# 0411tony/Yue

Hardware: AMD Instinct MI355X
Metric: BPR triplet-updates/sec at k=128 (S-round semantics, user rows sequential; the reference's exact sequential semantics: secondary.exact) (higher is better)
Workload: dtype f32

## Files before the change

### yue_amd/csrc/bpr_host.hip

```cpp
#include "host_common.hpp"

#include "train_kernels.hpp"
#include "round_kernels.hpp"

using yue_host::fail;
using yue_host::kr_of;
using yue_host::with_kr;
static_assert(yue::kNllSlots == yue_host::kNllSlotsHost && yue::kHeaderSlack == yue_host::kHeaderSlackHost &&
              yue::kMetaStageMax == (uint32_t)yue_host::kMetaStageMaxHost, "host_common.hpp mirrors these");

namespace {

yue::TrainArgs make_args(yue_ctx *c, double lr, double regU, double regI) {
    yue::TrainArgs a{};
    a.P = c->P.p; a.Q = c->Q.p; a.dP = c->dP.p; a.dQ = c->dQ.p;
    a.stage = c->Q.p ? c->Q.p + (size_t)c->n * c->k : nullptr;
    a.ev_u = c->ev_u.p; a.ev_i = c->ev_i.p; a.ev_j = c->ev_j.p;
    a.indptr = c->indptr.p; a.indices = c->indices.p;
    a.nll_slots = c->scal.p;
    a.m = c->m; a.n = c->n; a.k = c->k;
    a.lr = lr;
    a.ru = (float)(lr * regU);
    a.ri = (float)(lr * regI);
    a.neg_lo = 0; a.neg_range = (int32_t)c->n;
    return a;
}

void launch_level(yue_ctx *c, const yue::TrainArgs &a, int64_t e0, int64_t e1) {
    const int tpw = (int)std::min<int64_t>(64, std::max<int64_t>(1, (e1 - e0) / 4096));
    const int64_t waves = (e1 - e0 + tpw - 1) / tpw;
    const dim3 grid((unsigned)((waves + 3) / 4)), block(256);
    with_kr(c->k, [&](auto kr) { hipLaunchKernelGGL(yue::k_bpr_level<kr()>, grid, block, 0, c->stream, a, e0, e1, tpw); });
}

constexpr int kRoundInstances[][2] = {{1, 8}, {1, 16}, {2, 8}, {4, 4}, {1, 4}, {2, 4}, {1, 2}, {2, 2}};

constexpr int default_round_tpw(int kr, bool meta) { return kr == 4 ? 4 : kr == 2 ? 8 : meta ? 8 : 16; }

template <class F, size_t... I>
bool with_round_instance(int kr, int tpw, F &&f, std::index_sequence<I...>) {
    return ((kr == kRoundInstances[I][0] && tpw == kRoundInstances[I][1] &&
             (f(std::integral_constant<int, kRoundInstances[I][0]>{}, std::integral_constant<int, kRoundInstances[I][1]>{}), true)) || ...);
}
template <class F>
bool with_round_instance(int kr, int tpw, F &&f) {
    return with_round_instance(kr, tpw, f, std::make_index_sequence<sizeof kRoundInstances / sizeof kRoundInstances[0]>{});
}

int tpw_of(const yue_ctx *c, bool meta) { return c->opt_round_tpw ? c->opt_round_tpw : default_round_tpw(kr_of(c->k), meta); }

constexpr int64_t kMetaRangeMax = 37 * 1024;
constexpr int64_t kMetaRangesMax = 12;
constexpr int64_t kRoundGenerationsMax = 6;
constexpr double kRoundEventsPerItemRow = 4.0;

bool meta_bucketed(const yue_ctx *c) { return c->n > kMetaRangeMax * kMetaRangesMax || c->opt_round_bucket; }
bool meta_path_fits(const yue_ctx *c) { return c->opt_round_meta && c->n <= ((int64_t)yue::kBucketRangesMax << yue::kBucketShift); }

int default_round_events(yue_ctx *c, double n_rows, int64_t *out) {
    const bool fold = yue_host::fold_path(c);
    const int tpw = tpw_of(c, fold);
    int per_cu = 0, cus = 0;
    hipError_t e = hipSuccess;
    if (!with_round_instance(kr_of(c->k), tpw, [&](auto kr, auto t) {
            e = fold ? hipOccupancyMaxActiveBlocksPerMultiprocessor(&per_cu, yue::k_round_m<kr(), t()>, 256, 0)
                     : hipOccupancyMaxActiveBlocksPerMultiprocessor(&per_cu, yue::k_round<kr(), t()>, 256, 0);
        }))
        return fail(YUE_ERR_ARG, "unsupported (k, TPW) combination");
    HIPCHK(e);
    per_cu = std::min(per_cu, fold ? 7 : 6);
    HIPCHK(hipDeviceGetAttribute(&cus, hipDeviceAttributeMultiprocessorCount, c->device));
    const double slots = (double)per_cu * (double)cus;
    int64_t w = (int64_t)(slots * 4.0 * tpw);
    w -= w % 1024;
    w = std::max<int64_t>(w, 1024);
    if (fold) {
        int64_t sets = std::min<int64_t>(kRoundGenerationsMax, std::max<int64_t>(1, (int64_t)(kRoundEventsPerItemRow * n_rows / (double)w)));
        if (2.0 * (double)(w * sets) < 2.0 * n_rows) sets = std::min<int64_t>(sets, 4);
        w *= sets;
    }
    *out = w;
    return YUE_OK;
}

int launch_round(yue_ctx *c, const yue::TrainArgs &a_in, int64_t e0, int64_t e1, int64_t n0, int64_t n1,
                 int parity, int apply_p) {
    unsigned long long *cnt[2] = {c->cnt0.p, c->cnt1.p};
    uint32_t *cntp[2] = {c->cntp0.p, c->cntp1.p};
    yue::RoundArgs ra{};
    ra.e_begin = e0; ra.e_end = e1; ra.n_begin = n0; ra.n_end = n1;
    ra.cnt_cur = cnt[parity]; ra.cnt_next = cnt[parity ^ 1]; ra.cntp_cur = cntp[parity]; ra.cntp_next = cntp[parity ^ 1];
    uint32_t *tab[2] = {c->tab0.p, c->tab1.p};
    ra.tab_cur = tab[parity]; ra.tab_next = tab[parity ^ 1]; ra.staged = c->staged ? 1 : 0;
    ra.apply_p = apply_p;
    const int tpw = tpw_of(c, false);
    const int64_t waves = (std::max(e1 - e0, n1 - n0) + tpw - 1) / tpw;
    const int64_t blocks = (waves + 3) / 4;
    if (blocks == 0) return YUE_OK;
    const dim3 grid((unsigned)blocks), block(256);
#ifdef YUE_STAMPS
    yue::TrainArgs a = a_in;
    a.stamps = nullptr;
    if (e1 > e0 && c->update_launches++ == c->stamp_launch) {
        HIPCHK(c->stamps.resize((size_t)waves * 8));
        HIPCHK(hipMemsetAsync(c->stamps.p, 0, (size_t)waves * 64, c->stream));
        a.stamps = c->stamps.p;
        c->stamp_waves = (e1 - e0 + tpw - 1) / tpw;
    }
#else
    const yue::TrainArgs &a = a_in;
#endif
    if (!with_round_instance(kr_of(c->k), tpw, [&](auto kr, auto t) {
            hipLaunchKernelGGL((yue::k_round<kr(), t()>), grid, block, 0, c->stream, a, ra, a.ev_u, a.ev_i, a.ev_j);
        }))
        return fail(YUE_ERR_ARG, "unsupported (k, TPW) combination");
    return YUE_OK;
}

int launch_round_meta(yue_ctx *c, const yue::TrainArgs &a, const std::vector<int64_t> &bounds) {
    const int64_t R = (int64_t)bounds.size() - 1;
    const int64_t E = bounds.back();
    HIPCHK(c->meta_i.resize((size_t)E + yue::kHeaderSlack)); HIPCHK(c->meta_j.resize((size_t)E + yue::kHeaderSlack));
    HIPCHK(c->round_rows.resize((size_t)R)); HIPCHK(c->d_bounds.resize((size_t)R + 1));
    if (c->h_bounds != bounds) {
        HIPCHK(hipStreamSynchronize(c->stream));
        c->h_bounds = bounds;
        HIPCHK(hipMemcpyAsync(c->d_bounds.p, c->h_bounds.data(), (size_t)(R + 1) * sizeof(int64_t), hipMemcpyHostToDevice, c->stream));
    }
    HIPCHK(hipMemsetAsync(c->round_rows.p, 0, (size_t)R * sizeof(unsigned long long), c->stream));
    HIPCHK(c->fold.resize((size_t)(E + 4 * R + 8)));
    yue::MetaArgs ma{};
    ma.ev_i = a.ev_i; ma.ev_j = a.ev_j; ma.bounds = c->d_bounds.p; ma.R = R; ma.n = (int32_t)c->n;
    const bool bucketed = meta_bucketed(c);
    if (bucketed) {
        ma.range = 1 << yue::kBucketShift;
        ma.G = (int32_t)((c->n + ma.range - 1) >> yue::kBucketShift);
        HIPCHK(c->bk_touch.resize((size_t)(2 * E + 2))); HIPCHK(c->bk_ptr.resize((size_t)R * (ma.G + 1)));
        yue::BucketArgs ba{};
        ba.ev_i = a.ev_i; ba.ev_j = a.ev_j; ba.bounds = c->d_bounds.p; ba.R = R; ba.G = ma.G;
        ba.bk_touch = c->bk_touch.p; ba.bk_ptr = c->bk_ptr.p; ba.meta_i = c->meta_i.p; ba.meta_j = c->meta_j.p;
        int cus0 = 0;
        HIPCHK(hipDeviceGetAttribute(&cus0, hipDeviceAttributeMultiprocessorCount, c->device));
        hipLaunchKernelGGL(yue::k_round_bucket, dim3((unsigned)std::min<int64_t>(R, 2 * cus0)), dim3(1024), 0, c->stream, ba);
        ma.bk_touch = c->bk_touch.p; ma.bk_ptr = c->bk_ptr.p;
    } else {
        ma.G = (int32_t)((c->n + kMetaRangeMax - 1) / kMetaRangeMax);
        ma.range = (int32_t)((c->n + ma.G - 1) / ma.G);
    }
    ma.chunk = (ma.range + 1023) / 1024; ma.chunk |= 1;
    int64_t widest = 0;
    for (int64_t r = 0; r < R; ++r) widest = std::max(widest, bounds[(size_t)r + 1] - bounds[(size_t)r]);
    const double mean_touches = 2.0 * (double)widest / (double)std::max<int64_t>(1, c->n);
    const uint32_t stage_auto = (uint32_t)std::min<double>((double)yue::kMetaStageMax, std::max<double>((double)yue::kMetaStageDefault,
                                                         std::ceil(mean_touches * (kr_of(c->k) == 1 ? 4.0 : 2.0))));
    ma.stage_max = !c->staged ? 1u : c->opt_round_stage >= 2 ? (uint32_t)c->opt_round_stage : stage_auto;
    c->last_stage_max = (int)ma.stage_max;
    ma.meta_i = c->meta_i.p; ma.meta_j = c->meta_j.p; ma.round_rows = c->round_rows.p; ma.fold = c->fold.p;
    const size_t lds = (size_t)ma.range * sizeof(uint32_t);
    const void *kfn = bucketed ? (const void *)yue::k_round_meta<true> : (const void *)yue::k_round_meta<false>;
    HIPCHK(hipFuncSetAttribute(kfn, hipFuncAttributeMaxDynamicSharedMemorySize, (int)lds));
    int per_cu = 0, cus = 0;
    if (bucketed) { HIPCHK(hipOccupancyMaxActiveBlocksPerMultiprocessor(&per_cu, yue::k_round_meta<true>, 1024, lds)); }
    else { HIPCHK(hipOccupancyMaxActiveBlocksPerMultiprocessor(&per_cu, yue::k_round_meta<false>, 1024, lds)); }
    HIPCHK(hipDeviceGetAttribute(&cus, hipDeviceAttributeMultiprocessorCount, c->device));
    const int64_t grid = std::max<int64_t>(8, std::min<int64_t>((R * ma.G + 7) / 8 * 8, (int64_t)std::max(per_cu, 1) * cus / 8 * 8));
    if (bucketed) hipLaunchKernelGGL(yue::k_round_meta<true>, dim3((unsigned)grid), dim3(1024), lds, c->stream, ma);
    else
        hipLaunchKernelGGL(yue::k_round_meta<false>, dim3((unsigned)grid), dim3(1024), lds, c->stream, ma);
    HIPCHK(hipGetLastError());
    return YUE_OK;
}

void launch_round_fold(yue_ctx *c, const yue::TrainArgs &a, int64_t e0, int64_t e1, int64_t round_index) {
    yue::FoldArgs f{};
    f.fold = c->fold.p + yue::fold_base(e0, round_index); f.round_rows = c->round_rows.p + round_index; f.Q = a.Q; f.dQ = a.dQ; f.stage = a.stage; f.k = c->k; f.capacity = (uint32_t)((e1 - e0) & ~(int64_t)3);
    const dim3 fgrid((unsigned)std::min<int64_t>(c->opt_fold_blocks, std::max<int64_t>(1, (e1 - e0 + 15) / 16))), block(256);
    with_kr(c->k, [&](auto kr) { hipLaunchKernelGGL(yue::k_round_fold<kr()>, fgrid, block, 0, c->stream, f); });
}

int launch_round_m(yue_ctx *c, const yue::TrainArgs &a_in, int64_t e0, int64_t e1, int64_t round_index) {
    yue::RoundMArgs ra{};
    ra.e_begin = e0; ra.e_end = e1; ra.staged = c->staged ? 1 : 0;
    const int tpw = tpw_of(c, true);
    const int64_t waves = (e1 - e0 + tpw - 1) / tpw;
    const int64_t blocks = (waves + 3) / 4;
    if (blocks == 0) return YUE_OK;
    const dim3 grid((unsigned)blocks), block(256);
#ifdef YUE_STAMPS
    yue::TrainArgs a = a_in;
    a.stamps = nullptr;
    if (c->update_launches++ == c->stamp_launch) {
        HIPCHK(c->stamps.resize((size_t)waves * 8));
        HIPCHK(hipMemsetAsync(c->stamps.p, 0, (size_t)waves * 64, c->stream));
        a.stamps = c->stamps.p;
        c->stamp_waves = waves;
    }
#else
    const yue::TrainArgs &a = a_in;
#endif
    const uint32_t *mi = c->meta_i.p, *mj = c->meta_j.p;
    if (c->bigq) {
        bool is_default = false;
        with_round_instance(kr_of(c->k), tpw, [&](auto kr, auto t) {
            if constexpr (t() == default_round_tpw(kr(), true)) {
// ... 8 lines not shown
        return fail(YUE_ERR_ARG, "unsupported (k, TPW) combination");
    launch_round_fold(c, a, e0, e1, round_index);
    return YUE_OK;
}

int launch_round_u(yue_ctx *c, const yue::TrainArgs &a, int64_t u0, int64_t u1, int64_t e0, int64_t e1, int64_t round_index) {
    yue::RoundUArgs ra{};
    ra.u_begin = u0; ra.u_end = u1; ra.ev_ptr = c->d_ev_ptr.p; ra.e_begin = e0; ra.e_end = e1; ra.staged = c->staged ? 1 : 0; ra.margins = c->margins.p;
    ra.psq_slots = c->psq_in_rounds ? c->psq_slots.p : nullptr;
    const int64_t blocks = (u1 - u0 + 3) / 4;
    if (blocks == 0) return YUE_OK;
    const dim3 grid((unsigned)blocks), block(256);
    const uint32_t *mi = c->meta_i.p, *mj = c->meta_j.p;
    with_kr(c->k, [&](auto kr) {
        if (c->opt_round_fast) hipLaunchKernelGGL((yue::k_round_u<kr(), true>), grid, block, 0, c->stream, a, ra, a.ev_i, a.ev_j, mi, mj);
        else hipLaunchKernelGGL((yue::k_round_u<kr(), false>), grid, block, 0, c->stream, a, ra, a.ev_i, a.ev_j, mi, mj);
    });
    launch_round_fold(c, a, e0, e1, round_index);
    return YUE_OK;
}

template <typename F>
int run_rounds(yue_ctx *c, yue::TrainArgs a, const std::vector<int64_t> &bounds, int apply_p, F after_round, bool meta = false, const std::vector<int64_t> *user_blocks = nullptr) {
    const int64_t R = (int64_t)bounds.size() - 1;
    int64_t widest = 0;
    for (int64_t r = 0; r < R; ++r) widest = std::max(widest, bounds[(size_t)r + 1] - bounds[(size_t)r]);
    if (widest >= (1ll << 24)) meta = false;
    const bool fits31 = (c->n + 2 * widest) * (int64_t)c->k * 4 < (1ll << 31);
    c->bigq = meta && !fits31;
    if (!meta && (int64_t)c->n * c->k * 4 >= (1ll << 31))
        return fail(YUE_ERR_ARG, "item matrices of 2 GiB and more per GPU are supported by yue_bpr_epoch's default path only (not by explicit rounds / round_meta = 0 / rounds of 2^24 events and more)");
    c->staged = c->opt_round_stage && widest > 0 && (fits31 || c->bigq);
    if (c->staged) {
        const size_t need = (size_t)(c->n + 2 * widest) * (size_t)c->k;
        if (c->Q.n < need) {
            DevBuf<float> bigger;
            HIPCHK(bigger.resize(need));
            HIPCHK(hipMemcpyAsync(bigger.p, c->Q.p, (size_t)c->n * c->k * sizeof(float), hipMemcpyDeviceToDevice, c->stream));
            HIPCHK(hipStreamSynchronize(c->stream));
            c->Q.release();
            c->Q = bigger;
            a.Q = c->Q.p;
        }
        if (!meta) {
            HIPCHK(c->tab0.resize((size_t)c->n * yue::kStageMax));
            HIPCHK(c->tab1.resize((size_t)c->n * yue::kStageMax));
        }
        a.stage = c->Q.p + (size_t)c->n * c->k;
    }
    std::vector<int64_t> ne;
    for (int64_t r = 0; r < R; ++r) if (bounds[(size_t)r + 1] > bounds[(size_t)r]) ne.push_back(r);
    int rc;
    if (meta) {
        if (!ne.empty() && (rc = launch_round_meta(c, a, bounds))) return rc;
    } else if (!ne.empty()) {
        const int64_t r0 = ne[0];
        if ((rc = launch_round(c, a, 0, 0, bounds[(size_t)r0], bounds[(size_t)r0 + 1], 1, apply_p))) return rc;
    }
    const bool timed = c->timing_stride > 0 && !ne.empty();
    if (timed) {
        if (c->ev_used == c->ev_pool.size()) {
            hipEvent_t s, t;
            HIPCHK(hipEventCreate(&s));
            HIPCHK(hipEventCreate(&t));
            c->ev_pool.emplace_back(s, t);
            c->ev_triplets.push_back(0);
            c->ev_launches.push_back(0);
        }
        HIPCHK(hipEventRecord(c->ev_pool[c->ev_used].first, c->stream));
    }
    size_t pos = 0;
    for (int64_t r = 0; r < R; ++r) {
        if (pos < ne.size() && ne[pos] == r) {
            const int64_t e0 = bounds[(size_t)r], e1 = bounds[(size_t)r + 1];
            int64_t n0 = 0, n1 = 0;
            if (pos + 1 < ne.size()) { n0 = bounds[(size_t)ne[pos + 1]]; n1 = bounds[(size_t)ne[pos + 1] + 1]; }
            const bool seq_user = meta && user_blocks && !c->bigq;
            if ((rc = seq_user ? launch_round_u(c, a, (*user_blocks)[(size_t)r], (*user_blocks)[(size_t)r + 1], e0, e1, r)
                      : meta ? launch_round_m(c, a, e0, e1, r) : launch_round(c, a, e0, e1, n0, n1, (int)(pos & 1), apply_p))) return rc;
            ++pos;
        }
        if ((rc = after_round(r))) return rc;
    }
    if (timed) {
        HIPCHK(hipEventRecord(c->ev_pool[c->ev_used].second, c->stream));
        c->ev_triplets[c->ev_used] = bounds.back() - bounds.front();
        c->ev_launches[c->ev_used] = (int64_t)ne.size();
        c->ev_used++;
    }
    return YUE_OK;
}

void reset_round_state(yue_ctx *c) {
    (void)hipStreamSynchronize(c->stream);
    if (c->cnt0.p) (void)hipMemsetAsync(c->cnt0.p, 0, c->cnt0.n * sizeof(unsigned long long), c->stream);
    if (c->cnt1.p) (void)hipMemsetAsync(c->cnt1.p, 0, c->cnt1.n * sizeof(unsigned long long), c->stream);
    if (c->cntp0.p) (void)hipMemsetAsync(c->cntp0.p, 0, c->cntp0.n * sizeof(uint32_t), c->stream);
    if (c->cntp1.p) (void)hipMemsetAsync(c->cntp1.p, 0, c->cntp1.n * sizeof(uint32_t), c->stream);
    if (c->dP.p) (void)hipMemsetAsync(c->dP.p, 0, c->dP.n * sizeof(float), c->stream);
    if (c->dQ.p) (void)hipMemsetAsync(c->dQ.p, 0, c->dQ.n * sizeof(float), c->stream);
    (void)hipStreamSynchronize(c->stream);
}

}

namespace yue_host {
bool fold_path(const yue_ctx *c) { return meta_path_fits(c); }
// ... 155 lines not shown
    HIPCHK(hipStreamSynchronize(c->stream));
    return YUE_OK;
}

int yue_adam_reset(yue_ctx *c) {
    if (!c || !c->have_factors) return fail(YUE_ERR_ARG, "yue_adam_reset: no factors uploaded");
    HIPCHK(hipSetDevice(c->device));
    const size_t mk = (size_t)c->m * c->k, nk = (size_t)c->n * c->k;
    HIPCHK(c->aU_m.resize(mk)); HIPCHK(c->aU_v.resize(mk)); HIPCHK(c->aV_m.resize(nk)); HIPCHK(c->aV_v.resize(nk));
    HIPCHK(hipMemsetAsync(c->aU_m.p, 0, mk * sizeof(float), c->stream)); HIPCHK(hipMemsetAsync(c->aU_v.p, 0, mk * sizeof(float), c->stream));
    HIPCHK(hipMemsetAsync(c->aV_m.p, 0, nk * sizeof(float), c->stream)); HIPCHK(hipMemsetAsync(c->aV_v.p, 0, nk * sizeof(float), c->stream));
    HIPCHK(hipMemsetAsync(c->dP.p, 0, mk * sizeof(float), c->stream)); HIPCHK(hipMemsetAsync(c->dQ.p, 0, nk * sizeof(float), c->stream));
    c->adam_m = c->m; c->adam_n = c->n; c->adam_k = c->k;
    return YUE_OK;
}

int yue_adam_get_moments(yue_ctx *c, float *mU, float *vU, float *mV, float *vV) {
    if (!c || !c->have_factors || c->adam_m != c->m || c->adam_n != c->n || c->adam_k != c->k)
        return fail(YUE_ERR_ARG, "yue_adam_get_moments: no Adam state for the uploaded factors");
    HIPCHK(hipSetDevice(c->device));
    HIPCHK(hipStreamSynchronize(c->stream));
    const size_t mk = (size_t)c->m * c->k * sizeof(float), nk = (size_t)c->n * c->k * sizeof(float);
    if (mU) HIPCHK(hipMemcpy(mU, c->aU_m.p, mk, hipMemcpyDeviceToHost));
    if (vU) HIPCHK(hipMemcpy(vU, c->aU_v.p, mk, hipMemcpyDeviceToHost));
    if (mV) HIPCHK(hipMemcpy(mV, c->aV_m.p, nk, hipMemcpyDeviceToHost));
    if (vV) HIPCHK(hipMemcpy(vV, c->aV_v.p, nk, hipMemcpyDeviceToHost));
    return YUE_OK;
}

int yue_adam_step(yue_ctx *c, const int32_t *u, const int32_t *i, const int32_t *j, int64_t T, double lr, double reg, int64_t step, double *loss_out) {
    if (!c || !c->have_factors) return fail(YUE_ERR_ARG, "yue_adam_step: no factors uploaded");
    if (T <= 0 || !u || !i || !j || step < 1) return fail(YUE_ERR_ARG, "yue_adam_step: bad argument (T > 0, step >= 1)");
    HIPCHK(hipSetDevice(c->device));
    if (c->adam_m != c->m || c->adam_n != c->n || c->adam_k != c->k) { const int rc0 = yue_adam_reset(c); if (rc0) return rc0; }
    for (int64_t t = 0; t < T; ++t)
        if (u[t] < 0 || u[t] >= c->m || i[t] < 0 || i[t] >= c->n || j[t] < 0 || j[t] >= c->n) return fail(YUE_ERR_ARG, "yue_adam_step: triplet " + std::to_string(t) + " out of range");
    int rc = upload_triplets(c, u, i, j, T, true);
    if (rc) return rc;
    if ((rc = zero_scalars(c))) return rc;
    yue::MbArgs a{};
    a.U = c->P.p; a.V = c->Q.p; a.gU = c->dP.p; a.gV = c->dQ.p; a.k = c->k; a.u = c->xu.p; a.i = c->xi.p; a.j = c->xj.p; a.T = T;
    a.reg = (float)reg; a.loss_slots = c->scal.p;
    const dim3 grid((unsigned)(((T + 31) / 32 + 3) / 4));
    with_kr(c->k, [&](auto kr) { hipLaunchKernelGGL(yue::k_mb_grad<kr()>, grid, dim3(256), 0, c->stream, a); });
    if ((rc = yue_host::adam_apply(c, lr, step))) return rc;
    return read_scalars(c, loss_out, nullptr, nullptr);
}

int yue_sample_negatives(yue_ctx *c, uint64_t seed, uint32_t epoch, int32_t *j_out) {
    if (!c || !c->have_inter || !j_out) return fail(YUE_ERR_ARG, "yue_sample_negatives: no interactions uploaded");
    HIPCHK(hipSetDevice(c->device));
    yue::TrainArgs a = make_args(c, 0, 0, 0);
    a.seed = seed; a.epoch = epoch;
    if (c->E > 0) {
        hipLaunchKernelGGL(yue::k_sample, dim3((unsigned)((c->E + 255) / 256)), dim3(256), 0, c->stream, a, c->E);
        HIPCHK(hipGetLastError());
        HIPCHK(hipMemcpyAsync(j_out, c->ev_j.p, c->E * sizeof(int32_t), hipMemcpyDeviceToHost, c->stream));
    }
    HIPCHK(hipStreamSynchronize(c->stream));
    return YUE_OK;
}

int yue_sumsq(yue_ctx *c, double *sp, double *sq) {
    if (!c || !c->have_factors) return fail(YUE_ERR_ARG, "yue_sumsq: no factors uploaded");
    HIPCHK(hipSetDevice(c->device));
    int rc = sumsq_async(c);
    if (rc) return rc;
    double h[2];
    HIPCHK(hipMemcpyAsync(h, c->scal.p + yue::kNllSlots + 1, sizeof h, hipMemcpyDeviceToHost, c->stream));
    HIPCHK(hipStreamSynchronize(c->stream));
    if (sp) *sp = h[0];
    if (sq) *sq = h[1];
    return YUE_OK;
}

int yue_bpr_epoch(yue_ctx *c, uint64_t seed, uint32_t epoch, int64_t round_events, double lr, double regU, double regI,
                  double *nll_out, double *sumsqP_out, double *sumsqQ_out) {
    if (!c || !c->have_factors || !c->have_inter) return fail(YUE_ERR_ARG, "yue_bpr_epoch: upload factors and interactions first");
    if (round_events < 0) return fail(YUE_ERR_ARG, "yue_bpr_epoch: round_events must be positive (or 0 for the device's default)");
    HIPCHK(hipSetDevice(c->device));
    yue::TrainArgs a = make_args(c, lr, regU, regI);
    a.seed = seed + 0x632BE59BD9B4E019ull * (uint64_t)c->rank;
    a.epoch = epoch;
    int rc = zero_scalars(c);
    if (rc) return rc;
    const int64_t E = c->E;
    if (E > 0) hipLaunchKernelGGL(yue::k_sample, dim3((unsigned)((E + 255) / 256)), dim3(256), 0, c->stream, a, E);
    if (c->opt_epoch_exact) {
        if (yue_host::on_communicator(c) && c->nranks > 1) return fail(YUE_ERR_ARG, "yue_bpr_epoch: option epoch_exact runs on one GPU (the sequential order spans all item shards)");
        if ((rc = yue_host::chain_epoch(c, lr, regU, regI))) return rc;
        if ((rc = sumsq_async(c))) return rc;
        return read_scalars(c, nll_out, sumsqP_out, sumsqQ_out);
    }
    std::vector<int64_t> bounds;
    double tot[2] = {(double)E, (double)c->n};
    if (yue_host::on_communicator(c)) {
        if ((rc = yue_allreduce_f64(c, tot, 2))) return rc;
        if ((rc = zero_scalars(c))) return rc;
    }
    const double etot = tot[0];
    if (round_events == 0 && (rc = default_round_events(c, tot[1] / c->nranks, &round_events))) return rc;
    int64_t ub = 1, group = 1;
    if ((rc = yue_epoch_plan(c->m, c->k, round_events, etot, c->nranks, &ub, &group, nullptr))) return rc;
    if (!yue_host::on_communicator(c)) group = std::max<int64_t>(1, (c->m + ub - 1) / ub);
    else group = std::max<int64_t>(1, ((int64_t)c->opt_comm_group_mb << 20) / std::max<int64_t>(1, ub * c->k * 4));
    std::vector<int64_t> ublock;
    for (int64_t u0 = 0; u0 < c->m; u0 += ub) { ublock.push_back(u0); bounds.push_back(c->h_ev_ptr[(size_t)u0]); }
    ublock.push_back(c->m); bounds.push_back(E);
    const int64_t R = (int64_t)ublock.size() - 1;
    const bool seq_user = !yue_host::on_communicator(c) && c->opt_round_user_seq && meta_path_fits(c);
    if (seq_user) {
        HIPCHK(c->d_ev_ptr.resize((size_t)c->m + 1));
        if (!c->d_ev_ptr_valid) {
            HIPCHK(hipMemcpyAsync(c->d_ev_ptr.p, c->h_ev_ptr.data(), ((size_t)c->m + 1) * sizeof(int64_t), hipMemcpyHostToDevice, c->stream));
            c->d_ev_ptr_valid = true;
        }
        HIPCHK(c->margins.resize((size_t)std::max<int64_t>(E, 1)));
    }
    c->psq_in_rounds = seq_user && c->all_users_have_events && E > 0;
    if (c->psq_in_rounds) {
        HIPCHK(c->psq_slots.resize((size_t)yue::kNllSlots));
        HIPCHK(hipMemsetAsync(c->psq_slots.p, 0, (size_t)yue::kNllSlots * sizeof(double), c->stream));
    }
    c->last_round_user_seq = 0;
    auto after = [&](int64_t r) -> int {
        if (seq_user && !c->bigq) { c->last_round_user_seq = 1; return YUE_OK; }
        if ((r + 1) % group != 0 && r + 1 != R) return YUE_OK;
        const int64_t g_first = ublock[(size_t)(r - (r % group))], g_last = ublock[(size_t)r + 1];
        const int64_t first = g_first * c->k, count = (g_last - g_first) * c->k;
        const dim3 grid((unsigned)std::min<int64_t>(4096, (count + 255) / 256));
        if (!yue_host::on_communicator(c)) {
            hipLaunchKernelGGL(yue::k_apply_range, grid, dim3(256), 0, c->stream, c->P.p, c->dP.p, first, count);
            return YUE_OK;
        }
        HIPCHK(hipEventRecord(c->ev_rounds, c->stream));
        HIPCHK(hipStreamWaitEvent(c->comm_stream, c->ev_rounds, 0));
        c->comm_collectives += 1;
        c->comm_bytes += (double)count * sizeof(float);
        if (const int rcr = yue_host::reduce_user_block(c, first, count, c->comm_stream)) return rcr;
        hipLaunchKernelGGL(yue::k_apply_range, grid, dim3(256), 0, c->comm_stream, c->P.p, c->dP.p, first, count);
        return YUE_OK;
    };
    c->comm_collectives = 0; c->comm_bytes = 0.0; c->comm_wait_ms = 0.0;
    if ((rc = run_rounds(c, a, bounds, 0, after, meta_path_fits(c), seq_user ? &ublock : nullptr))) { reset_round_state(c); return rc; }
    if (c->last_round_user_seq && E > 0)
        hipLaunchKernelGGL(yue::k_loss_margins, dim3(2048), dim3(256), 0, c->stream, c->margins.p, c->ev_j.p, E, c->scal.p);
    const bool psq_done = c->psq_in_rounds && c->last_round_user_seq;
    c->psq_in_rounds = false;
    if (yue_host::on_communicator(c)) {
        HIPCHK(hipEventRecord(c->ev_t_rounds, c->stream));
        HIPCHK(hipEventRecord(c->ev_t_comm, c->comm_stream));
    }
    HIPCHK(hipEventRecord(c->ev_comm, c->comm_stream));
    HIPCHK(hipStreamWaitEvent(c->stream, c->ev_comm, 0));
    c->comm_compute_waits = 1;
    HIPCHK(hipGetLastError());
    if ((rc = sumsq_async(c, psq_done ? c->psq_slots.p : nullptr))) return rc;
    if ((rc = read_scalars(c, nll_out, sumsqP_out, sumsqQ_out))) return rc;
    if (yue_host::on_communicator(c)) {
        float ms = 0.f;
        HIPCHK(hipEventSynchronize(c->ev_t_comm));
        HIPCHK(hipEventElapsedTime(&ms, c->ev_t_rounds, c->ev_t_comm));
        c->comm_wait_ms = ms > 0.f ? ms : 0.0;
    }
    return YUE_OK;
}

int yue_epoch_plan(int64_t m, int k, int64_t round_events, double events_total, int nranks,
                   int64_t *user_block, int64_t *blocks_per_group, int64_t *n_blocks) {
// ... 60 lines not shown
```

### yue_amd/csrc/host_common.hpp

```cpp
#pragma once
#include "../../include/yue_hip.h"

#include <hip/hip_runtime.h>

#include <algorithm>
#include <cmath>
#include <cstdio>
#include <cstdlib>
#include <cstring>
#include <string>
#include <type_traits>
#include <vector>

struct ncclComm;
struct yue_wrmf;
struct yue_knn;
struct yue_expo;
struct yue_cof;
struct yue_cnet;
struct yue_s2v;
struct yue_lgcn;
struct yue_ngcf;
struct yue_cdae;
struct yue_ipf;
// ... 62 lines not shown
    DevBuf<uint2> fold, bk_touch;
    DevBuf<uint32_t> bk_ptr;
    DevBuf<int64_t> d_bounds;
    std::vector<int64_t> h_bounds;
#ifdef YUE_STAMPS
    DevBuf<unsigned long long> stamps;
    int64_t stamp_launch = -1, update_launches = 0, stamp_waves = 0;
#endif
    DevBuf<int32_t> ev_u, ev_i, ev_j, indices;
    DevBuf<int64_t> indptr;
    DevBuf<int32_t> xu, xi, xj, xk;
    DevBuf<double> x_loss;
    DevBuf<float> aU_m, aU_v, aV_m, aV_v;
    int64_t adam_m = 0, adam_n = 0; int adam_k = 0;
    DevBuf<double> scal;
    std::vector<int64_t> h_ev_ptr;
    bool all_users_have_events = false;
    bool psq_in_rounds = false;
    DevBuf<int32_t> s_users, s_ids, s_mask_idx, s_flags;
    DevBuf<int32_t> s_few, s_few_ids;
    DevBuf<float> s_few_scores;
    int64_t scan_few_users = 0;
    DevBuf<int64_t> s_mask_ptr;
    DevBuf<float> s_scores, s_row, s_norms;
    double scan_ms = 0.0;
    int64_t scan_events = 0, scan_rescored = 0, scan_tiles_done = 0, scan_tiles_total = 0;
    DevBuf<unsigned long long> s_work;
    DevBuf<unsigned short> s_qb;
    DevBuf<uint32_t> s_masks;
    int opt_scan_two_phase = 1;
    int64_t opt_scan_streams_min_users = 262144;
    int opt_scan_slabs = 4;
    int opt_scan_streams = 2;
    int opt_scan_filter_ub = 3;
    int opt_scan_growth = 0;
    int scan_chunks = 0;
    int scan_used_bf16 = 0;
    int opt_scan_f32 = 0;
    int opt_scan_batch = 0;
    int opt_round_tpw = 0;
    int opt_topn_true = 0;
    int scan_settle = 0;
    int last_stage_max = 0;
    int opt_round_stage = 1;
    int opt_round_bucket = 0;
    int opt_fold_blocks = 1536;
    int opt_round_user_seq = 1;
    int opt_round_fast = 1;
    int last_round_user_seq = 0;
    int opt_comm_group_mb = 8;
    int opt_round_cus_reserved = 0;
    int64_t comm_compute_waits = 0;
    int opt_round_meta = 1;
    int timing_stride = 0;
    std::vector<std::pair<hipEvent_t, hipEvent_t>> ev_pool;
    std::vector<int64_t> ev_triplets, ev_launches;
    size_t ev_used = 0;
    DevBuf<double> fP, fBi, f_coef, f_x, f_hist, f_scores, f_out_sc;
    DevBuf<float> fQ;
    DevBuf<int64_t> f_ptr;
    DevBuf<int32_t> f_items, f_negs, f_ids, f_flags;
    DevBuf<int64_t> f_uq_ptr, f_neg_ptr;
    DevBuf<int32_t> f_uq_items, f_loc_i, f_loc_j;
    DevBuf<float> f_wq, f_dQ;
    DevBuf<double> f_wp, f_wb, f_dP, f_dB;
    DevBuf<unsigned> f_cnt;
    int64_t fn = 0;
    int fk = 0;
    int opt_fism_inplace = 1;
    int opt_fism_lds = 1;
    DevBuf<uint32_t> ch_key, ch_val, ch_key2, ch_val2, ch_seg, ch_ord_i, ch_ord_j, ch_head, ch_incl, ch_ord_u, ch_rkey, ch_rval;
    DevBuf<int64_t> ch_run_ptr, d_ev_ptr;
    DevBuf<int32_t> ch_run_u;
    DevBuf<unsigned char> ch_tmp;
    DevBuf<unsigned> ch_Qv, ch_Pv;
    DevBuf<unsigned long long> ch_ctl;
    DevBuf<unsigned long long> ch_stats;
    bool d_ev_ptr_valid = false;
    int opt_epoch_exact = 0;
    int opt_replay_levels = 0;
    int opt_chain_split = -1;
    int opt_chain_ring = 0;
    int opt_chain_xcd = 0;
    int opt_chain_fast = 0;
    int opt_chain_waves = 0;
    int64_t opt_chain_spin = 0;
    int64_t chain_runs = 0, chain_waves = 0, chain_groups = 0, chain_kernel_us = 0, replay_levels = 0;
    hipEvent_t ev_chain0 = nullptr, ev_chain1 = nullptr;
    ncclComm *comm = nullptr;
    int rank = 0, nranks = 1;
    hipStream_t comm_stream = nullptr;
    hipEvent_t ev_rounds = nullptr, ev_comm = nullptr;
    hipEvent_t ev_t_rounds = nullptr, ev_t_comm = nullptr;
    int (*seam_reduce)(void *host, int64_t count, int dtype, void *user) = nullptr;
    void *seam_user = nullptr;
    std::vector<float> seam_buf;
    int64_t comm_collectives = 0;
    double comm_bytes = 0.0, comm_wait_ms = 0.0;
    int comm_version = 0, comm_nranks_reported = 0;
    hipEvent_t ev_scan0 = nullptr, ev_scan1 = nullptr;
    yue_wrmf *wrmf = nullptr;
    yue_knn *knn = nullptr;
    yue_ipf *ipf = nullptr;
    yue_expo *expo = nullptr;
    yue_cof *cof = nullptr;
    yue_cnet *cnet = nullptr;
// ... 62 lines not shown
```

### yue_amd/csrc/options_host.hip

```cpp
#include "host_common.hpp"

#include <limits>

using yue_host::fail;

namespace {

struct Option {
    const char *name;
    int64_t (*get)(yue_ctx *);
    void (*put)(yue_ctx *, int64_t);
    int (*set)(const Option &, yue_ctx *, int64_t);
    int64_t lo, hi;
    const char *refusal;
    std::vector<int64_t> also;
};
#define YUE_AT(member) [](yue_ctx *c) -> int64_t { return c->member; }, [](yue_ctx *c, int64_t v) { c->member = (decltype(c->member))v; }

int set_flag(const Option &o, yue_ctx *c, int64_t value) { o.put(c, value != 0); return YUE_OK; }

int set_ranged(const Option &o, yue_ctx *c, int64_t value) {
    if ((value < o.lo || value > o.hi) && std::find(o.also.begin(), o.also.end(), value) == o.also.end())
        return fail(YUE_ERR_ARG, std::string("yue_set_option: ") + o.name + " " + o.refusal);
    o.put(c, value);
// ... 11 lines not shown
    hipStream_t fresh = nullptr;
    if (value == 0) HIPCHK(hipStreamCreateWithFlags(&fresh, hipStreamNonBlocking));
    else {
        std::vector<uint32_t> mask((size_t)(cus + 31) / 32, 0u);
        for (int cu = 0; cu < cus - (int)value; ++cu) mask[(size_t)cu / 32] |= 1u << (cu % 32);
        HIPCHK(hipExtStreamCreateWithCUMask(&fresh, (uint32_t)mask.size(), mask.data()));
    }
    (void)hipStreamDestroy(c->stream);
    c->stream = fresh;
    c->opt_round_cus_reserved = (int)value;
    return YUE_OK;
}

int set_round_tpw(const Option &, yue_ctx *c, int64_t value) {
    if (value != 0 && value != 2 && value != 4 && value != 8 && value != 16) return fail(YUE_ERR_ARG, "yue_set_option: round_tpw must be 0, 2, 4, 8 or 16");
    if (value == 8 && yue_host::kr_of(c->k) == 4) return fail(YUE_ERR_ARG, "yue_set_option: round_tpw 8 needs k <= 128");
    if (value == 16 && yue_host::kr_of(c->k) != 1) return fail(YUE_ERR_ARG, "yue_set_option: round_tpw 16 needs k <= 64");
    c->opt_round_tpw = (int)value;
    return YUE_OK;
}

#ifdef YUE_STAMPS
int set_stamp_launch(const Option &, yue_ctx *c, int64_t value) { c->stamp_launch = value; c->update_launches = 0; return YUE_OK; }
#endif

const Option kOptions[] = {
    {"scan_f32", YUE_AT(opt_scan_f32), set_flag},
    {"scan_batch", YUE_AT(opt_scan_batch), set_ranged, 0, 1, "must be 0 or 1"},
    {"scan_two_phase", YUE_AT(opt_scan_two_phase), set_flag},
    {"scan_growth", YUE_AT(opt_scan_growth), set_ranged, 2, 64, "must be 0 (automatic) or 2..64", {0}},
    {"scan_filter_ub", YUE_AT(opt_scan_filter_ub), set_ranged, 1, 3, "must be 1, 2 or 3"},
    {"scan_streams", YUE_AT(opt_scan_streams), set_ranged, 1, 2, "must be 1 or 2"},
    {"scan_slabs", YUE_AT(opt_scan_slabs), set_ranged, 2, 64, "must be 2..64"},
    {"scan_streams_min_users", YUE_AT(opt_scan_streams_min_users), set_ranged, 1024, std::numeric_limits<int64_t>::max(), "must be at least 1024"},
    {"scan_last_chunks", YUE_AT(scan_chunks)},
    {"scan_last_few_users", YUE_AT(scan_few_users)},
    {"scan_last_settle", YUE_AT(scan_settle)},
    {"topn_true", YUE_AT(opt_topn_true), set_flag},
    {"fism_lds", YUE_AT(opt_fism_lds), set_flag},
    {"fism_inplace", YUE_AT(opt_fism_inplace), set_flag},
    {"round_stage", YUE_AT(opt_round_stage), set_ranged, 0, yue_host::kMetaStageMaxHost, "must be 0, 1 or 2..64"},
    {"round_last_stage_max", YUE_AT(last_stage_max)},
    {"round_meta", YUE_AT(opt_round_meta), set_flag},
    {"comm_group_mb", YUE_AT(opt_comm_group_mb), set_ranged, 1, 4096, "must be 1..4096"},
    {"round_cus_reserved", YUE_AT(opt_round_cus_reserved), set_round_cus_reserved},
    {"comm_last_compute_waits", YUE_AT(comm_compute_waits)},
    {"round_user_seq", YUE_AT(opt_round_user_seq), set_flag},
    {"round_fast", YUE_AT(opt_round_fast), set_flag},
    {"round_last_user_seq", YUE_AT(last_round_user_seq)},
    {"round_bucket", YUE_AT(opt_round_bucket), set_flag},
    {"fold_blocks", YUE_AT(opt_fold_blocks), set_ranged, 1, 65536, "out of range"},
    {"round_tpw", YUE_AT(opt_round_tpw), set_round_tpw},
    {"round_path", round_path},
#ifdef YUE_STAMPS
    {"debug_stamp_launch", nullptr, nullptr, set_stamp_launch},
#endif
    {"epoch_exact", YUE_AT(opt_epoch_exact), set_flag},
    {"replay_levels", YUE_AT(opt_replay_levels), set_flag},
    {"chain_waves", YUE_AT(opt_chain_waves), set_ranged, 0, 8, "must be 0..8"},
    {"chain_split", YUE_AT(opt_chain_split), set_ranged, -1, 1, "must be -1, 0 or 1"},
    {"chain_fast", YUE_AT(opt_chain_fast), set_flag},
    {"chain_xcd", YUE_AT(opt_chain_xcd), set_flag},
    {"chain_ring", YUE_AT(opt_chain_ring), set_ranged, 0, 0, "must be 0, 8 or 16", {8, 16}},
    {"chain_spin", YUE_AT(opt_chain_spin), set_ranged, 0, 0x7fffffff, "out of range"},
    {"chain_last_us", YUE_AT(chain_kernel_us)},
    {"chain_last_runs", YUE_AT(chain_runs)},
    {"chain_last_waves", YUE_AT(chain_waves)},
    {"replay_last_levels", YUE_AT(replay_levels)},
    {"lgcn_hub", YUE_AT(opt_lgcn_hub), set_ranged, 1, 0x7fffffff, "must be 1 .. 2^31 - 1"},
    {"lgcn_last_hubs", YUE_AT(lgcn_hubs)},
    {"lgcn_last_parts", YUE_AT(lgcn_parts)},
    {"lgcn_last_forward_ns", YUE_AT(lgcn_ns[0])},
    {"lgcn_last_batch_ns", YUE_AT(lgcn_ns[1])},
    {"lgcn_last_backward_ns", YUE_AT(lgcn_ns[2])},
    {"lgcn_last_adam_ns", YUE_AT(lgcn_ns[3])},
    {"ngcf_hub", YUE_AT(opt_ngcf_hub), set_ranged, 1, 0x7fffffff, "must be 1 .. 2^31 - 1"},
    {"ngcf_last_hubs", YUE_AT(ngcf_hubs)},
    {"ngcf_last_parts", YUE_AT(ngcf_parts)},
    {"ngcf_last_gather_ns", YUE_AT(ngcf_ns[0])},
    {"ngcf_last_dense_ns", YUE_AT(ngcf_ns[1])},
    {"ngcf_last_batch_ns", YUE_AT(ngcf_ns[2])},
    {"ngcf_last_backward_ns", YUE_AT(ngcf_ns[3])},
    {"ngcf_last_wgrad_ns", YUE_AT(ngcf_ns[4])},
    {"ngcf_last_adam_ns", YUE_AT(ngcf_ns[5])},
    {"cdae_hub", YUE_AT(opt_cdae_hub), set_ranged, 1, 0x7fffffff, "must be 1 .. 2^31 - 1"},
    {"cdae_last_hubs", YUE_AT(cdae_hubs)},
    {"cdae_last_parts", YUE_AT(cdae_parts)},
    {"cdae_last_saturated", YUE_AT(cdae_saturated)},
};
#undef YUE_AT

const Option *find_option(const std::string &key) {
    for (const Option &o : kOptions) if (key == o.name) return &o;
    return nullptr;
}

}

extern "C" {

int yue_get_option(yue_ctx *c, const char *name, int64_t *value) {
    if (!c || !name || !value) return fail(YUE_ERR_ARG, "yue_get_option: null argument");
    const std::string key(name);
    const Option *o = find_option(key);
    if (o && o->get) { *value = o->get(c); return YUE_OK; }
    if (key.compare(0, 5, "wrmf_") == 0) return yue_host::wrmf_get_option(c, key, value);
// ... 26 lines not shown
```

### yue_amd/csrc/train_kernels.hpp

```cpp
#pragma once
#include "bpr_device.hpp"

namespace yue {

__global__ void __launch_bounds__(256) k_sample(TrainArgs a, int64_t E) {
    int64_t e = (int64_t)blockIdx.x * blockDim.x + threadIdx.x;
    if (e < E) a.ev_j[e] = sample_negative(a, a.ev_u[e], e);
}

template <int KR>
__global__ void __launch_bounds__(256) k_bpr_level(TrainArgs a, int64_t e_begin, int64_t e_end, int tpw) {
    const int lane = threadIdx.x & 63;
    const int64_t wave = (int64_t)blockIdx.x * (blockDim.x >> 6) + (threadIdx.x >> 6);
    const int64_t base = e_begin + wave * tpw;
    if (base >= e_end) return;
    const int cnt = (int)((e_end - base) < (int64_t)tpw ? (e_end - base) : (int64_t)tpw);
    int u = 0, i = 0, j = 0;
    if (lane < cnt) { u = a.ev_u[base + lane]; i = a.ev_i[base + lane]; j = a.ev_j[base + lane]; }
    const int k = a.k;
    double nll = 0.0;
    for (int t = 0; t < cnt; ++t) {
        const int64_t tu = __builtin_amdgcn_readlane(u, t);
        const int64_t ti = __builtin_amdgcn_readlane(i, t);
        const int64_t tj = __builtin_amdgcn_readlane(j, t);
        float p[KR], qi[KR], qj[KR];
#pragma unroll
        for (int r = 0; r < KR; ++r) {
            const int e = 64 * r + lane;
            p[r] = e < k ? a.P[tu * k + e] : 0.0f;
            qi[r] = e < k ? a.Q[ti * k + e] : 0.0f;
            qj[r] = e < k ? a.Q[tj * k + e] : 0.0f;
        }
        float ai = 0.0f, aj = 0.0f;
#pragma unroll
        for (int r = 0; r < KR; ++r) { const float a1 = p[r] * qi[r]; ai = ai + a1; const float a2 = p[r] * qj[r]; aj = aj + a2; }
        const float x = wave_sum(ai) - wave_sum(aj);
        const double s = 1.0 / (1.0 + exp(-(double)x));
        const float c = (float)(a.lr * (1.0 - s));
        nll += -log(s);
#pragma unroll
        for (int r = 0; r < KR; ++r) {
            const int e = 64 * r + lane;
            const Elem o = bpr_elem(p[r], qi[r], qj[r], c, a.ru, a.ri);
            if (e < k) { a.P[tu * k + e] = o.p2; a.Q[ti * k + e] = o.qi2; a.Q[tj * k + e] = o.qj2; }
        }
    }
    if (lane == 0) atomicAdd(a.nll_slots + (wave & (kNllSlots - 1)), nll);
}

struct MbArgs {
    const float *U, *V;
    float *gU, *gV;
    int k;
    const int32_t *u, *i, *j;
    int64_t T;
    float reg;
    double *loss_slots;
};

template <int KR>
// ... 452 lines not shown
```

Measured before the change: 1.789 billion.

## Sample negatives per user wave with register-resident rows and cross-lane search

Adds a user-centric negative-sampling kernel, on by default, in which each wave handles four users. Each user's positive-item row is loaded into registers across lanes, and membership of a candidate is tested by a cross-lane binary search using ds_bpermute, replacing per-triplet global-memory searches of the CSR row. Rows longer than 256 items fall back to the old per-event sampler. Also hoists the widest-round computation out of launch_round_meta and adds options for the sampling form and negative range; the added risks are kernel complexity and load imbalance on heavy users.

```diff
diff --git a/yue_amd/csrc/bpr_host.hip b/yue_amd/csrc/bpr_host.hip
--- a/yue_amd/csrc/bpr_host.hip
+++ b/yue_amd/csrc/bpr_host.hip
@@ -24,6 +24,27 @@
     a.ri = (float)(lr * regI);
     a.neg_lo = 0; a.neg_range = (int32_t)c->n;
     return a;
+}
+
+int ensure_ev_ptr(yue_ctx *c) {
+    HIPCHK(c->d_ev_ptr.resize((size_t)c->m + 1));
+    if (!c->d_ev_ptr_valid) {
+        HIPCHK(hipMemcpyAsync(c->d_ev_ptr.p, c->h_ev_ptr.data(), ((size_t)c->m + 1) * sizeof(int64_t), hipMemcpyHostToDevice, c->stream));
+        c->d_ev_ptr_valid = true;
+    }
+    return YUE_OK;
+}
+
+int launch_sample(yue_ctx *c, const yue::TrainArgs &a) {
+    if (c->E <= 0) return YUE_OK;
+    if (c->opt_sample_form == 0) {
+        hipLaunchKernelGGL(yue::k_sample, dim3((unsigned)((c->E + 255) / 256)), dim3(256), 0, c->stream, a, c->E);
+        return YUE_OK;
+    }
+    if (const int rc = ensure_ev_ptr(c)) return rc;
+    const int64_t waves = (c->m + yue::kSampleUsers - 1) / yue::kSampleUsers;
+    hipLaunchKernelGGL(yue::k_sample_u, dim3((unsigned)((waves + 3) / 4)), dim3(256), 0, c->stream, a, c->d_ev_ptr.p);
+    return YUE_OK;
 }
 
 void launch_level(yue_ctx *c, const yue::TrainArgs &a, int64_t e0, int64_t e1) {
@@ -117,7 +138,7 @@
     return YUE_OK;
 }
 
-int launch_round_meta(yue_ctx *c, const yue::TrainArgs &a, const std::vector<int64_t> &bounds) {
+int launch_round_meta(yue_ctx *c, const yue::TrainArgs &a, const std::vector<int64_t> &bounds, int64_t widest) {
     const int64_t R = (int64_t)bounds.size() - 1;
     const int64_t E = bounds.back();
     HIPCHK(c->meta_i.resize((size_t)E + yue::kHeaderSlack)); HIPCHK(c->meta_j.resize((size_t)E + yue::kHeaderSlack));
@@ -148,8 +169,6 @@
         ma.range = (int32_t)((c->n + ma.G - 1) / ma.G);
     }
     ma.chunk = (ma.range + 1023) / 1024; ma.chunk |= 1;
-    int64_t widest = 0;
-    for (int64_t r = 0; r < R; ++r) widest = std::max(widest, bounds[(size_t)r + 1] - bounds[(size_t)r]);
     const double mean_touches = 2.0 * (double)widest / (double)std::max<int64_t>(1, c->n);
     const uint32_t stage_auto = (uint32_t)std::min<double>((double)yue::kMetaStageMax, std::max<double>((double)yue::kMetaStageDefault,
                                                          std::ceil(mean_touches * (kr_of(c->k) == 1 ? 4.0 : 2.0))));
@@ -264,7 +283,7 @@
     for (int64_t r = 0; r < R; ++r) if (bounds[(size_t)r + 1] > bounds[(size_t)r]) ne.push_back(r);
     int rc;
     if (meta) {
-        if (!ne.empty() && (rc = launch_round_meta(c, a, bounds))) return rc;
+        if (!ne.empty() && (rc = launch_round_meta(c, a, bounds, widest))) return rc;
     } else if (!ne.empty()) {
         const int64_t r0 = ne[0];
         if ((rc = launch_round(c, a, 0, 0, bounds[(size_t)r0], bounds[(size_t)r0 + 1], 1, apply_p))) return rc;
@@ -526,8 +545,12 @@
     HIPCHK(hipSetDevice(c->device));
     yue::TrainArgs a = make_args(c, 0, 0, 0);
     a.seed = seed; a.epoch = epoch;
+    if (c->opt_sample_neg_range) {
+        if ((int64_t)c->opt_sample_neg_lo + c->opt_sample_neg_range > c->n) return fail(YUE_ERR_ARG, "yue_sample_negatives: sample_neg_lo + sample_neg_range exceed the item count");
+        a.neg_lo = c->opt_sample_neg_lo; a.neg_range = c->opt_sample_neg_range;
+    }
     if (c->E > 0) {
-        hipLaunchKernelGGL(yue::k_sample, dim3((unsigned)((c->E + 255) / 256)), dim3(256), 0, c->stream, a, c->E);
+        if (const int rc = launch_sample(c, a)) return rc;
         HIPCHK(hipGetLastError());
         HIPCHK(hipMemcpyAsync(j_out, c->ev_j.p, c->E * sizeof(int32_t), hipMemcpyDeviceToHost, c->stream));
     }
@@ -559,7 +582,7 @@
     int rc = zero_scalars(c);
     if (rc) return rc;
     const int64_t E = c->E;
-    if (E > 0) hipLaunchKernelGGL(yue::k_sample, dim3((unsigned)((E + 255) / 256)), dim3(256), 0, c->stream, a, E);
+    if ((rc = launch_sample(c, a))) return rc;
     if (c->opt_epoch_exact) {
         if (yue_host::on_communicator(c) && c->nranks > 1) return fail(YUE_ERR_ARG, "yue_bpr_epoch: option epoch_exact runs on one GPU (the sequential order spans all item shards)");
         if ((rc = yue_host::chain_epoch(c, lr, regU, regI))) return rc;
@@ -584,11 +607,7 @@
     const int64_t R = (int64_t)ublock.size() - 1;
     const bool seq_user = !yue_host::on_communicator(c) && c->opt_round_user_seq && meta_path_fits(c);
     if (seq_user) {
-        HIPCHK(c->d_ev_ptr.resize((size_t)c->m + 1));
-        if (!c->d_ev_ptr_valid) {
-            HIPCHK(hipMemcpyAsync(c->d_ev_ptr.p, c->h_ev_ptr.data(), ((size_t)c->m + 1) * sizeof(int64_t), hipMemcpyHostToDevice, c->stream));
-            c->d_ev_ptr_valid = true;
-        }
+        if ((rc = ensure_ev_ptr(c))) return rc;
         HIPCHK(c->margins.resize((size_t)std::max<int64_t>(E, 1)));
     }
     c->psq_in_rounds = seq_user && c->all_users_have_events && E > 0;
diff --git a/yue_amd/csrc/host_common.hpp b/yue_amd/csrc/host_common.hpp
--- a/yue_amd/csrc/host_common.hpp
+++ b/yue_amd/csrc/host_common.hpp
@@ -138,6 +138,8 @@
     int opt_round_cus_reserved = 0;
     int64_t comm_compute_waits = 0;
     int opt_round_meta = 1;
+    int opt_sample_form = 1;
+    int opt_sample_neg_lo = 0, opt_sample_neg_range = 0;
     int timing_stride = 0;
     std::vector<std::pair<hipEvent_t, hipEvent_t>> ev_pool;
     std::vector<int64_t> ev_triplets, ev_launches;
diff --git a/yue_amd/csrc/options_host.hip b/yue_amd/csrc/options_host.hip
--- a/yue_amd/csrc/options_host.hip
+++ b/yue_amd/csrc/options_host.hip
@@ -87,6 +87,9 @@
     {"fold_blocks", YUE_AT(opt_fold_blocks), set_ranged, 1, 65536, "out of range"},
     {"round_tpw", YUE_AT(opt_round_tpw), set_round_tpw},
     {"round_path", round_path},
+    {"sample_form", YUE_AT(opt_sample_form), set_ranged, 0, 1, "must be 0 or 1"},
+    {"sample_neg_lo", YUE_AT(opt_sample_neg_lo), set_ranged, 0, std::numeric_limits<int32_t>::max(), "must be 0 .. 2^31 - 1"},
+    {"sample_neg_range", YUE_AT(opt_sample_neg_range), set_ranged, 0, std::numeric_limits<int32_t>::max(), "must be 0 (all items) .. 2^31 - 1"},
 #ifdef YUE_STAMPS
     {"debug_stamp_launch", nullptr, nullptr, set_stamp_launch},
 #endif
diff --git a/yue_amd/csrc/train_kernels.hpp b/yue_amd/csrc/train_kernels.hpp
--- a/yue_amd/csrc/train_kernels.hpp
+++ b/yue_amd/csrc/train_kernels.hpp
@@ -6,6 +6,79 @@
 __global__ void __launch_bounds__(256) k_sample(TrainArgs a, int64_t E) {
     int64_t e = (int64_t)blockIdx.x * blockDim.x + threadIdx.x;
     if (e < E) a.ev_j[e] = sample_negative(a, a.ev_u[e], e);
+}
+
+constexpr int kSampleUsers = 4;
+constexpr int kSampleRowMax = 256;
+
+__device__ __forceinline__ int32_t lane_read(int32_t v, int src_lane) { return __builtin_amdgcn_ds_bpermute(src_lane << 2, v); }
+
+template <int RPL>
+__device__ __forceinline__ bool row_contains(const int32_t (&row)[RPL], int32_t c) {
+    int pos = 0;
+#pragma unroll
+    for (int s = 32; s > 0; s >>= 1) pos += lane_read(row[RPL - 1], pos + s - 1) < c ? s : 0;
+    bool found = false;
+#pragma unroll
+    for (int q = 0; q < RPL; ++q) found |= lane_read(row[q], pos) == c;
+    return found;
+}
+
+template <int RPL>
+__device__ __forceinline__ void sample_user(const TrainArgs &a, int lane, const int32_t (&row)[RPL], int64_t e0, int64_t e1) {
+    for (int64_t base = e0; base < e1; base += 64) {
+        const int64_t e = base + lane;
+        const bool mine = e < e1;
+        bool pending = mine;
+        int32_t j = -1;
+        for (uint32_t t = 0; t < (uint32_t)kMaxAttempts && __builtin_amdgcn_ballot_w64(pending) != 0ull; ++t) {
+            const int32_t c = ctr_draw(a.seed, a.epoch, (uint64_t)e, t, a.neg_lo, a.neg_range);
+            const bool taken = row_contains<RPL>(row, c);
+            if (pending && !taken) { j = c; pending = false; }
+        }
+        if (mine) a.ev_j[e] = j;
+    }
+}
+
+template <int RPL>
+__device__ __forceinline__ void load_row(int32_t (&row)[RPL], const int32_t *indices, int64_t lo, int len, int lane) {
+#pragma unroll
+    for (int q = 0; q < RPL; ++q) row[q] = RPL * lane + q < len ? indices[lo + RPL * lane + q] : INT32_MAX;
+}
+
+__global__ void __launch_bounds__(256) k_sample_u(TrainArgs a, const int64_t *__restrict__ ev_ptr) {
+    const int lane = threadIdx.x & 63;
+    const int64_t u0 = (int64_t)__builtin_amdgcn_readfirstlane((int)(blockIdx.x * 4u + (threadIdx.x >> 6))) * kSampleUsers;
+    if (u0 >= a.m) return;
+    const int users = (int)(a.m - u0 < kSampleUsers ? a.m - u0 : kSampleUsers);
+    const int64_t my = u0 + (lane < users ? lane : users);
+    const int64_t ip = a.indptr[my], ep = ev_ptr[my];
+    int64_t lo[kSampleUsers + 1], e0[kSampleUsers + 1];
+#pragma unroll
+    for (int q = 0; q <= kSampleUsers; ++q) {
+        lo[q] = ((int64_t)__builtin_amdgcn_readlane((int)(ip >> 32), q) << 32) | (uint32_t)__builtin_amdgcn_readlane((int)ip, q);
+        e0[q] = ((int64_t)__builtin_amdgcn_readlane((int)(ep >> 32), q) << 32) | (uint32_t)__builtin_amdgcn_readlane((int)ep, q);
+    }
+    int32_t row1[kSampleUsers][1];
+#pragma unroll
+    for (int q = 0; q < kSampleUsers; ++q) {
+        const int len = q < users ? (int)(lo[q + 1] - lo[q] < 65 ? lo[q + 1] - lo[q] : 65) : 0;
+        row1[q][0] = INT32_MAX;
+        if (len <= 64) load_row<1>(row1[q], a.indices, lo[q], e0[q + 1] > e0[q] ? len : 0, lane);
+    }
+#pragma unroll
+    for (int q = 0; q < kSampleUsers; ++q) {
+        if (q >= users || e0[q + 1] <= e0[q]) continue;
+        const int64_t len = lo[q + 1] - lo[q];
+        if (len <= 64) sample_user<1>(a, lane, row1[q], e0[q], e0[q + 1]);
+        else if (len <= kSampleRowMax) {
+            int32_t row4[4];
+            load_row<4>(row4, a.indices, lo[q], (int)len, lane);
+            sample_user<4>(a, lane, row4, e0[q], e0[q + 1]);
+        } else {
+            for (int64_t e = e0[q] + lane; e < e0[q + 1]; e += 64) a.ev_j[e] = sample_negative(a, (int32_t)(u0 + q), e);
+        }
+    }
 }
 
 template <int KR>
```

After: 1.804 billion (median of 6 runs). Within noise of the previous version (+0.9%).
